# ypw0102/GDR

Hardware: AMD Instinct MI355X
Metric: queries/sec on NQ-320k (768-d) (higher is better)
Workload: dtype f32; 1 GPU; C2/ragged/prefilter: t5-base encoder 512 q/GPU + Q.D^T top-100, 320000x768 corpus; batch_per_gpu=512, global_batch=512, seq_len=40, corpus_rows=320000, dim=768, k=100, encoder_rows=ragged

## Files before the change

### gdr_amd/csrc/common.h

```cpp
#pragma once
#include <hip/hip_runtime.h>
#include <stdint.h>
#include <stdio.h>
#include <stdarg.h>
#include <stdlib.h>

#include "../../include/gdr_hip.h"

namespace gdr {

void set_error(const char* fmt, ...);

#define GDR_CHECK_ARG(cond, ...)                \
  do {                                          \
    if (!(cond)) {                              \
      gdr::set_error(__VA_ARGS__);              \
      return GDR_EINVAL;                        \
    }                                           \
  } while (0)

void count_launch();
#define GDR_CHECK_LAUNCH(what)                                                   \
  do {                                                                           \
    gdr::count_launch();                                                         \
// ... 29 lines not shown
  ~ProfScope();
};

constexpr int CNT_STRIDE = 32;
struct SimEpilogue {
  float* cand_val;
  int32_t* cand_idx;
  int32_t* cand_cnt;
  const float* thr;
  int32_t* status;
  int32_t cap;
  int32_t tile_stride;
  int32_t mode;
};

struct StreamK {
  float* part;
  int32_t* flag;
  int32_t epoch;
  const int32_t* live = nullptr;
};
constexpr size_t STREAMK_PART_BYTES = (size_t)512 * 128 * 128 * 4;
constexpr size_t STREAMK_BYTES = STREAMK_PART_BYTES + 4096;

enum { ACT_NONE = 0, ACT_RELU = 1, ACT_GELU = 2 };
struct LinearEpilogue {
  bool has_bias, has_residual;
  int act;
};
static inline bool decode_epilogue(int epilogue, LinearEpilogue* e) {
  if (epilogue < GDR_EPI_NONE || epilogue > GDR_EPI_BIAS_GELU) return false;
  e->has_bias = epilogue == GDR_EPI_BIAS || epilogue == GDR_EPI_BIAS_RELU || epilogue == GDR_EPI_BIAS_RESIDUAL ||
                epilogue == GDR_EPI_BIAS_GELU;
  e->has_residual = epilogue == GDR_EPI_RESIDUAL || epilogue == GDR_EPI_BIAS_RESIDUAL;
  e->act = (epilogue == GDR_EPI_RELU || epilogue == GDR_EPI_BIAS_RELU) ? ACT_RELU
           : epilogue == GDR_EPI_BIAS_GELU                             ? ACT_GELU
                                                                       : ACT_NONE;
  return true;
}

int launch_linear_f32(const float* A, int64_t lda, const float* W, int64_t ldw, float* C, int64_t ldc, int64_t M,
                      int N, int K, int epilogue, const float* bias, const float* residual, int64_t ldr,
                      hipStream_t stream);
int launch_linear_f32_ws(const float* A, int64_t lda, const float* W, int64_t ldw, float* C, int64_t ldc, int64_t M,
                         int N, int K, int epilogue, const float* bias, const float* residual, int64_t ldr,
                         float* splitk_ws, size_t splitk_ws_bytes, hipStream_t stream, StreamK* sk = nullptr,
                         const int64_t* m_dev = nullptr, int64_t prof_rows = -1);
int launch_linear_f32_ws_dev(const float* A, int64_t lda, const float* W, int64_t ldw, float* C, int64_t ldc, int64_t M_max,
                             const int64_t* m_dev, int N, int K, int epilogue, const float* bias, const float* residual,
                             int64_t ldr, float* splitk_ws, size_t splitk_ws_bytes, hipStream_t stream,
                             StreamK* sk = nullptr);
int launch_linear_f32_dev(const float* A, int64_t lda, const float* W, int64_t ldw, float* C, int64_t ldc, int64_t M_max,
                          const int64_t* m_dev, int N, int K, int epilogue, const float* bias, const float* residual,
                          int64_t ldr, int64_t prof_rows, hipStream_t stream, StreamK* sk = nullptr);
int launch_sim_gemm(const void* D, int64_t N, const void* Q, int B, int d, const SimEpilogue& ep, bool bf16,
                    hipStream_t stream);

int launch_linear_bf16(const void* A, int64_t lda, const void* W, int64_t ldw, float* C, int64_t ldc, int64_t M, int N,
                       int K, int epilogue, const float* bias, const float* residual, int64_t ldr, hipStream_t stream,
                       const int64_t* m_dev = nullptr);
struct NormEpilogue {
  int kind;
  const float *w1, *b1, *w2, *b2, *addv;
  float eps;
  float* Y;
  int64_t ldy;
  int y16_only = 0;
};
struct SlabRef {
  const float* part;
  int S, tiles_n;
};
int launch_linear_f32_small(const float* A, int64_t lda, const float* W, int64_t ldw, float* C, int64_t ldc, int64_t M, int N,
                            int K, int has_bias, int has_residual, int act, const float* bias, const float* residual,
                            int64_t ldr, float* ws, size_t ws_bytes, hipStream_t stream, const int64_t* m_dev = nullptr,
                            const NormEpilogue* ne = nullptr,
                            SlabRef* slabs = nullptr,
                            const int32_t* live = nullptr);
int linear_f32_small_splits(int64_t M, int N, int K, bool has_ws, size_t ws_bytes);
int launch_linear_bf16_headdot(const void* A, int64_t lda, const void* W, int64_t ldw, int64_t M, const int64_t* m_dev, int N, int K,
                               const float* h, int64_t ldh, const int32_t* rows_map, const float* E, int dot_d, float scale,
                               float* partial, hipStream_t stream);
int linear_bf16_tile_form(int64_t M, int N, int K, int has_residual, int out_bf16, int split = 0);
int launch_linear_bf16_glds(const void* A, int64_t lda, const void* W, int64_t ldw, float* C, int64_t ldc, int64_t M, int N,
                            int K, int has_bias, int has_residual, int act, const float* bias, const float* residual,
                            int64_t ldr, int out_bf16, hipStream_t stream, const int64_t* m_dev = nullptr,
                            int split = 0);
int split_row_elems(int K, int f16x2 = 0);
int launch_split_f32_bf16x3(const float* in, int64_t ld_in, void* out, int64_t ld_out, int64_t rows, int K, const int64_t* rows_dev,
                            hipStream_t stream, int f16x2 = 0);
int launch_sim_bf16_glds(const void* D, int64_t N, const void* Q, int B, int d, const SimEpilogue& ep, int64_t n_doc_tiles,
                         hipStream_t stream);
int launch_cast_f32_bf16(const float* in, void* out_bf16, int64_t n, hipStream_t stream);

bool sim_stream_supported(int B, int d, bool bf16);
int launch_sim_stream(const void* D, int64_t N, const void* Q, int B, int d, const SimEpilogue& ep, bool bf16, hipStream_t stream);

template <int CTRL>
__device__ __forceinline__ float dpp_row(float v) {
  return __builtin_bit_cast(float, __builtin_amdgcn_update_dpp(0, __builtin_bit_cast(int, v), CTRL, 0xF, 0xF, false));
}
__device__ __forceinline__ float row16_sum(float v) {
  v += dpp_row<0x128>(v);
  v += dpp_row<0x124>(v);
  v += dpp_row<0x122>(v);
  v += dpp_row<0x121>(v);
  return v;
// ... 32 lines not shown
```

### gdr_amd/csrc/common.hip

```cpp
#include <atomic>

#include "common.h"

#include <mutex>
#include <vector>

namespace gdr {
static thread_local char g_err[512] = "";

void set_error(const char* fmt, ...) {
  va_list ap;
  va_start(ap, fmt);
  vsnprintf(g_err, sizeof(g_err), fmt, ap);
  va_end(ap);
}

namespace {
struct AttrKey {
  const void* fn;
  int dev;
};
std::mutex g_attr_mu;
std::vector<AttrKey> g_attr_done;
}

int ensure_dyn_lds(const void* kernel, int bytes, const char* what) {
  int dev = 0;
  if (hipGetDevice(&dev) != hipSuccess) {
    set_error("%s: hipGetDevice failed", what);
    return GDR_EHIP;
  }
  std::lock_guard<std::mutex> lock(g_attr_mu);
  for (const AttrKey& k : g_attr_done)
    if (k.fn == kernel && k.dev == dev) return GDR_OK;
  hipError_t e = hipFuncSetAttribute(kernel, hipFuncAttributeMaxDynamicSharedMemorySize, bytes);
  if (e != hipSuccess) {
    set_error("%s: hipFuncSetAttribute: %s", what, hipGetErrorString(e));
    return GDR_EHIP;
  }
  g_attr_done.push_back(AttrKey{kernel, dev});
  return GDR_OK;
}

struct ProfState {
  bool on = false;
  bool gate = true;
  int cap = 0, used = 0;
  hipEvent_t* start = nullptr;
  hipEvent_t* stop = nullptr;
  int* cls = nullptr;
  double* work = nullptr;
};
static ProfState g_prof;

ProfScope::ProfScope(int c, double w, hipStream_t s) : slot(-1), stream(s) {
  if (!g_prof.on || !g_prof.gate || g_prof.used >= g_prof.cap) return;
  slot = g_prof.used++;
  g_prof.cls[slot] = c;
  g_prof.work[slot] = w;
  (void)hipEventRecord(g_prof.start[slot], stream);
}
ProfScope::~ProfScope() {
  if (slot >= 0) (void)hipEventRecord(g_prof.stop[slot], stream);
}
}

extern "C" void gdr_prof_gate(int on) { gdr::g_prof.gate = on != 0; }

extern "C" int gdr_prof_enable(int max_events) {
  using namespace gdr;
  if (g_prof.on || max_events <= 0) {
    set_error("prof_enable: already enabled or bad size");
    return GDR_EINVAL;
  }
  g_prof.start = new hipEvent_t[max_events];
  g_prof.stop = new hipEvent_t[max_events];
  g_prof.cls = new int[max_events];
  g_prof.work = new double[max_events];
  for (int i = 0; i < max_events; ++i) {
    if (hipEventCreate(&g_prof.start[i]) != hipSuccess || hipEventCreate(&g_prof.stop[i]) != hipSuccess) {
      set_error("prof_enable: hipEventCreate failed");
      return GDR_EHIP;
    }
  }
  g_prof.cap = max_events, g_prof.used = 0, g_prof.on = true;
  return GDR_OK;
}

extern "C" int gdr_prof_collect(int64_t* launches, double* total_ms, double* total_work) {
  using namespace gdr;
  if (!g_prof.on) {
    set_error("prof_collect: profiler not enabled");
    return GDR_EINVAL;
  }
  for (int c = 0; c < PROF_NCLASS; ++c) launches[c] = 0, total_ms[c] = 0.0, total_work[c] = 0.0;
  int rc = GDR_OK;
  for (int i = 0; i < g_prof.used; ++i) {
    float ms = 0.f;
    if (hipEventSynchronize(g_prof.stop[i]) != hipSuccess ||
        hipEventElapsedTime(&ms, g_prof.start[i], g_prof.stop[i]) != hipSuccess) {
      set_error("prof_collect: event query failed");
      rc = GDR_EHIP;
      break;
    }
    const int c = g_prof.cls[i];
    launches[c] += 1, total_ms[c] += ms, total_work[c] += g_prof.work[i];
  }
  for (int i = 0; i < g_prof.cap; ++i) {
    (void)hipEventDestroy(g_prof.start[i]);
    (void)hipEventDestroy(g_prof.stop[i]);
  }
  delete[] g_prof.start, delete[] g_prof.stop, delete[] g_prof.cls, delete[] g_prof.work;
  g_prof = ProfState();
  return rc;
}

namespace gdr {
static std::atomic<int64_t> g_launches{0};
void count_launch() { g_launches.fetch_add(1, std::memory_order_relaxed); }
}
extern "C" int64_t gdr_launch_count(void) { return gdr::g_launches.load(std::memory_order_relaxed); }
extern "C" const char* gdr_last_error(void) { return gdr::g_err; }
extern "C" int gdr_abi_version(void) { return 9; }
```

### gdr_amd/csrc/encoder.hip

```cpp
#include <stdlib.h>

#include "layers.h"

namespace gdr {

constexpr size_t ENC_SPLITK_BYTES = (size_t)112 << 20;
static_assert(STREAMK_BYTES <= ENC_SPLITK_BYTES, "stream-K scratch must fit the split-K region");
constexpr bool ENC_LAST_Q_CLS_DEFAULT = true;

static int enc_streamk(char* splitk_region, StreamK* sk, hipStream_t stream) {
  sk->part = reinterpret_cast<float*>(splitk_region);
  sk->flag = reinterpret_cast<int32_t*>(splitk_region + STREAMK_PART_BYTES);
  sk->epoch = 0;
  if (hipMemsetAsync(sk->flag, 0, 512 * sizeof(int32_t), stream) != hipSuccess) {
    set_error("t5_encoder: memset of the stream-K flags failed");
    return GDR_EHIP;
  }
  return GDR_OK;
}

struct EncWs {
  size_t off_h, off_nx, off_qkv, off_ctx, off_ff, off_splitk, off_bf, total;
};

static EncWs enc_ws(const GdrT5Dims& dm, int64_t M, bool bf16 = false) {
  EncWs w{};
  const size_t inner = (size_t)dm.num_heads * dm.d_kv;
  size_t o = 0;
  w.off_h = o, o += align_up((size_t)M * dm.d_model * 4, 256);
  w.off_nx = o, o += align_up((size_t)M * dm.d_model * 4, 256);
  w.off_qkv = o, o += align_up((size_t)M * 3 * inner * 4, 256);
  w.off_ctx = o, o += align_up((size_t)M * inner * 4, 256);
  w.off_ff = o, o += align_up((size_t)M * dm.d_ff * 4, 256);
  w.off_splitk = o, o += ENC_SPLITK_BYTES;
  w.off_bf = o;
  if (bf16) o += align_up((size_t)M * (dm.d_ff > dm.d_model ? dm.d_ff : dm.d_model) * 2, 256);
  w.total = o;
  return w;
}

}

extern "C" size_t gdr_t5_encoder_workspace_bytes(const GdrT5Dims* dims, int B, int L) {
  if (!dims || B <= 0 || L <= 0) return 0;
  return gdr::enc_ws(*dims, (int64_t)B * L).total;
}

namespace gdr {
static int t5_encoder_impl(const GdrT5EncoderWeights* w, const int64_t* ids, const int64_t* mask, int B, int L,
                           float* out_hidden, float* out_pooled, void* workspace, size_t workspace_bytes, bool bf16,
                           hipStream_t stream) {
  if (B == 0) return GDR_OK;
  GDR_CHECK_ARG(w && ids && out_hidden && workspace, "t5_encoder: null pointer");
// ... 73 lines not shown
      at.out_bf16 = abf;
      if ((rc = launch_attention(at, stream))) return rc;
      if ((rc = lin16(abf, ly.wo, h, d, d, inner, 0, h, 0))) return rc;
      if ((rc = launch_rmsnorm_bf16(h, ly.ln_ff, abf, M, d, dm.eps, stream))) return rc;
      if ((rc = lin16(abf, ly.wi, ff, dm.d_ff, dm.d_ff, d, 1, nullptr, 1))) return rc;
      if ((rc = lin16(ff, ly.wo_ff, h, d, d, dm.d_ff, 0, h, 0))) return rc;
      continue;
    }
    if ((rc = launch_rmsnorm(h, ly.ln_attn, nx, M, d, dm.eps, nullptr, 1, stream))) return rc;
    if ((rc = linear(nx, d, ly.wqkv, qkv, 3 * inner, 3 * inner, d, GDR_EPI_NONE, nullptr))) return rc;
    if ((rc = launch_attention(at, stream))) return rc;
    if ((rc = linear(ctx, inner, ly.wo, h, d, d, inner, GDR_EPI_RESIDUAL, h))) return rc;
    if ((rc = launch_rmsnorm(h, ly.ln_ff, nx, M, d, dm.eps, nullptr, 1, stream))) return rc;
    if ((rc = linear(nx, d, ly.wi, ff, dm.d_ff, dm.d_ff, d, GDR_EPI_RELU, nullptr))) return rc;
    if ((rc = linear(ff, dm.d_ff, ly.wo_ff, h, d, d, dm.d_ff, GDR_EPI_RESIDUAL, h))) return rc;
  }
  return launch_rmsnorm(h, w->final_ln, out_hidden, M, d, dm.eps, out_pooled, L, stream);
}
}

extern "C" int gdr_t5_encoder_forward(const GdrT5EncoderWeights* w, const int64_t* ids, const int64_t* mask, int B,
                                      int L, float* out_hidden, float* out_pooled, void* workspace,
                                      size_t workspace_bytes, void* stream_) {
  return gdr::t5_encoder_impl(w, ids, mask, B, L, out_hidden, out_pooled, workspace, workspace_bytes, false,
                              static_cast<hipStream_t>(stream_));
}

namespace gdr {
struct RagWs {
  size_t seq_len, seq_off, row_src, rows_total, ctx_cls, h_cls, nx_cls, ff_cls, total;
};
static RagWs rag_ws(const GdrT5Dims& dm, int B, int L, size_t base) {
  RagWs r{};
  const size_t inner = (size_t)dm.num_heads * dm.d_kv;
  size_t o = base;
  r.seq_len = o, o += align_up((size_t)B * 4, 256);
  r.seq_off = o, o += align_up((size_t)(B + 1) * 4, 256);
  r.row_src = o, o += align_up((size_t)B * L * 4, 256);
  r.rows_total = o, o += 256;
  r.ctx_cls = o, o += align_up((size_t)B * inner * 4, 256);
  r.h_cls = o, o += align_up((size_t)B * dm.d_model * 4, 256);
  r.nx_cls = o, o += align_up((size_t)B * dm.d_model * 4, 256);
  r.ff_cls = o, o += align_up((size_t)B * dm.d_ff * 4, 256);
  r.total = o;
  return r;
}
static bool ragged_packs(const GdrT5Dims& dm, int B, int L) {
  const int64_t tiles = (((int64_t)B * L + 127) / 128) * ((dm.d_model + 127) / 128);
  return dm.d_kv == 64 && tiles >= 192 && dm.d_model % 32 == 0 && dm.d_ff % 32 == 0 && (dm.num_heads * dm.d_kv) % 32 == 0;
}
static bool ragged_packs_small(const GdrT5Dims& dm, int B, int L) {
  return dm.d_kv == 64 && (int64_t)B * L >= 256 && dm.d_model % 32 == 0 && dm.d_ff % 32 == 0 && (dm.num_heads * dm.d_kv) % 32 == 0;
}
}

extern "C" size_t gdr_t5_encoder_ragged_workspace_bytes(const GdrT5Dims* dims, int B, int L) {
  if (!dims || B <= 0 || L <= 0) return 0;
  return gdr::rag_ws(*dims, B, L, gdr::enc_ws(*dims, (int64_t)B * L, true).total).total;
}

namespace gdr {
static int ragged_impl(const GdrT5EncoderWeights* w, const int64_t* ids, const int64_t* mask, int B, int L, float* out_hidden,
                       float* out_pooled, int64_t live_rows_hint, void* workspace, size_t workspace_bytes, bool bf16,
                       hipStream_t stream) {
  if (B == 0) return GDR_OK;
  GDR_CHECK_ARG(w && ids && mask && workspace && (out_hidden || out_pooled), "t5_encoder_ragged: null pointer");
  const GdrT5Dims& dm = w->dims;
  GDR_CHECK_ARG(B > 0 && L > 0 && L <= T5_MAX_LEN, "t5_encoder_ragged: B=%d L=%d (L must be in [1,%d])", B, L, T5_MAX_LEN);
  GDR_CHECK_ARG(dm.d_model % 4 == 0 && dm.d_kv % 4 == 0 && dm.d_ff % 4 == 0, "t5_encoder_ragged: dims must be multiples of 4");
  GDR_CHECK_ARG(w->embed && w->rel_bias && w->final_ln && w->layers, "t5_encoder_ragged: null weight pointer");
  const int64_t M = (int64_t)B * L;
  const EncWs ws = enc_ws(dm, M, true);
  const RagWs rw = rag_ws(dm, B, L, ws.total);
  if (workspace_bytes < rw.total) {
    set_error("t5_encoder_ragged: workspace %zu < required %zu", workspace_bytes, rw.total);
    return GDR_ENOSPC;
  }
  GDR_CHECK_ARG(((uintptr_t)workspace & 255) == 0, "t5_encoder_ragged: workspace must be 256-byte aligned");
  char* base = static_cast<char*>(workspace);
  const int d = dm.d_model, H = dm.num_heads, dk = dm.d_kv, inner = H * dk;
  int rc;
  int32_t* seq_len = reinterpret_cast<int32_t*>(base + rw.seq_len);
  int32_t* seq_off = reinterpret_cast<int32_t*>(base + rw.seq_off);
  int32_t* row_src = reinterpret_cast<int32_t*>(base + rw.row_src);
  int64_t* rows_dev = reinterpret_cast<int64_t*>(base + rw.rows_total);
  if ((rc = launch_pack_plan(mask, B, L, seq_len, seq_off, row_src, rows_dev, stream))) return rc;
  const bool fused16 = bf16 && d % 64 == 0 && inner % 64 == 0 && dm.d_ff % 64 == 0 && (((uintptr_t)w->layers[0].wqkv) & 15) == 0;
  const bool big = ragged_packs(dm, B, L);
  const bool small = !big && !bf16 && ragged_packs_small(dm, B, L);
  if ((!big && !small) || (bf16 && !fused16)) {
    float* full = out_hidden ? out_hidden : reinterpret_cast<float*>(base + ws.off_qkv);
    if ((rc = t5_encoder_impl(w, ids, mask, B, L, full, out_pooled, workspace, ws.total, bf16, stream))) return rc;
    return out_hidden ? launch_zero_dead_rows(out_hidden, seq_len, B, L, d, stream) : GDR_OK;
  }
  if (bf16) {
    float* h = reinterpret_cast<float*>(base + ws.off_h);
    float* nx = reinterpret_cast<float*>(base + ws.off_nx);
    float* qkv = reinterpret_cast<float*>(base + ws.off_qkv);
    float* ff = reinterpret_cast<float*>(base + ws.off_ff);
    void* abf = base + ws.off_bf;
    float* h_cls = reinterpret_cast<float*>(base + rw.h_cls);
    void* ctx_cls16 = base + rw.ctx_cls;
    void* nx_cls16 = base + rw.nx_cls;
    void* ff_cls16 = base + rw.ff_cls;
    auto lin16 = [&](const void* A, const float* W, float* C, int64_t ldc, int64_t rows, const int64_t* md, int N, int K, int act,
                     const float* residual, int out_bf16) -> int {
      ProfScope prof(PROF_LINEAR, 2.0 * (double)(md && live_rows_hint >= 0 ? live_rows_hint : rows) * (double)N * (double)K, stream);
      const int rc_ = launch_linear_bf16_glds(A, K, W, K, C, ldc, rows, N, K, 0, residual != nullptr, act, nullptr, residual, ldc,
                                              out_bf16, stream, md);
      if (rc_ > 0) {
        set_error("t5_encoder_ragged_bf16: shape not served by the LDS-DMA linear");
        return GDR_EINVAL;
      }
      return rc_;
    };
    if ((rc = launch_embed_packed(w->embed, ids, row_src, rows_dev, M, d, dm.vocab_size, h, stream))) return rc;
    AttnArgs at{};
    const bool qkv16 = L <= 128;
    if (qkv16) {
      const __bf16* q16 = reinterpret_cast<const __bf16*>(qkv);
      at.q = reinterpret_cast<const float*>(q16), at.k = reinterpret_cast<const float*>(q16 + inner);
      at.v = reinterpret_cast<const float*>(q16 + 2 * inner), at.qkv_bf16 = 1;
    } else {
      at.q = qkv, at.k = qkv + inner, at.v = qkv + 2 * inner;
    }
    at.out = nullptr, at.out_bf16 = abf;
    at.ldq = at.ldk = at.ldv = 3 * inner, at.ldo = inner;
    at.q_bstride = at.k_bstride = at.o_bstride = L;
    at.B = B, at.H = H, at.dk = dk, at.Lq = L, at.Lk = L;
    at.q_pos0 = 0, at.scale = 1.0f;
    at.rel_bias = w->rel_bias, at.bidirectional = 1, at.num_buckets = dm.rel_buckets;
    at.lut = make_bucket_lut(dm.rel_buckets / 2, dm.rel_max_distance);
    at.key_mask = mask, at.mask_bstride = L, at.causal = 0, at.causal_neg_inf = 0;
    at.kv_rows = nullptr, at.kv_group = 1;
    at.seq_off = seq_off, at.seq_len = seq_len;
    const bool pooled_only = out_hidden == nullptr;
    for (int i = 0; i < dm.num_layers; ++i) {
      const GdrT5EncLayer& ly = w->layers[i];
      GDR_CHECK_ARG(ly.ln_attn && ly.wqkv && ly.wo && ly.ln_ff && ly.wi && ly.wo_ff, "t5_encoder_ragged: layer %d null weight", i);
      if ((rc = launch_rmsnorm_bf16_dev(h, ly.ln_attn, abf, rows_dev, M, d, dm.eps, stream))) return rc;
      if ((rc = lin16(abf, ly.wqkv, qkv, 3 * inner, M, rows_dev, 3 * inner, d, 0, nullptr, qkv16 ? 1 : 0))) return rc;
      if ((rc = launch_attention(at, stream))) return rc;
      if (pooled_only && i == dm.num_layers - 1) {
        if ((rc = launch_gather_rows(static_cast<const float*>(abf), seq_off, B, inner / 2, static_cast<float*>(ctx_cls16), stream)))
          return rc;
        if ((rc = launch_gather_rows(h, seq_off, B, d, h_cls, stream))) return rc;
        if ((rc = lin16(ctx_cls16, ly.wo, h_cls, d, B, nullptr, d, inner, 0, h_cls, 0))) return rc;
        if ((rc = launch_rmsnorm_bf16(h_cls, ly.ln_ff, nx_cls16, B, d, dm.eps, stream))) return rc;
        if ((rc = lin16(nx_cls16, ly.wi, static_cast<float*>(ff_cls16), dm.d_ff, B, nullptr, dm.d_ff, d, 1, nullptr, 1))) return rc;
        if ((rc = lin16(ff_cls16, ly.wo_ff, h_cls, d, B, nullptr, d, dm.d_ff, 0, h_cls, 0))) return rc;
        return launch_rmsnorm(h_cls, w->final_ln, out_pooled, B, d, dm.eps, nullptr, 1, stream);
      }
      if ((rc = lin16(abf, ly.wo, h, d, M, rows_dev, d, inner, 0, h, 0))) return rc;
      if ((rc = launch_rmsnorm_bf16_dev(h, ly.ln_ff, abf, rows_dev, M, d, dm.eps, stream))) return rc;
      if ((rc = lin16(abf, ly.wi, ff, dm.d_ff, M, rows_dev, dm.d_ff, d, 1, nullptr, 1))) return rc;
      if ((rc = lin16(ff, ly.wo_ff, h, d, M, rows_dev, d, dm.d_ff, 0, h, 0))) return rc;
    }
    if ((rc = launch_rmsnorm_dev(h, w->final_ln, nx, rows_dev, M, d, dm.eps, stream))) return rc;
    if (out_pooled && (rc = launch_gather_rows(nx, seq_off, B, d, out_pooled, stream))) return rc;
    if (out_hidden) {
      if (hipMemsetAsync(out_hidden, 0, (size_t)M * d * sizeof(float), stream) != hipSuccess) {
        set_error("t5_encoder_ragged: memset failed");
        return GDR_EHIP;
      }
      if ((rc = launch_scatter_rows(nx, row_src, rows_dev, M, d, out_hidden, stream))) return rc;
    }
    return GDR_OK;
  }
  float* h = reinterpret_cast<float*>(base + ws.off_h);
  float* nx = reinterpret_cast<float*>(base + ws.off_nx);
  float* qkv = reinterpret_cast<float*>(base + ws.off_qkv);
  float* ctx = reinterpret_cast<float*>(base + ws.off_ctx);
  float* ff = reinterpret_cast<float*>(base + ws.off_ff);
  float* ctx_cls = reinterpret_cast<float*>(base + rw.ctx_cls);
  float* h_cls = reinterpret_cast<float*>(base + rw.h_cls);
  float* nx_cls = reinterpret_cast<float*>(base + rw.nx_cls);
  float* ff_cls = reinterpret_cast<float*>(base + rw.ff_cls);
  StreamK sk{};
  if ((rc = enc_streamk(base + ws.off_splitk, &sk, stream))) return rc;
  float* skw = reinterpret_cast<float*>(base + ws.off_splitk);
  auto linear = [&](const float* A, int64_t lda, const float* W, float* C, int64_t ldc, int N, int K, int epi,
                    const float* residual) -> int {
    if (small)
      return launch_linear_f32_ws(A, lda, W, K, C, ldc, M, N, K, epi, nullptr, residual, ldc, skw, ENC_SPLITK_BYTES, stream, &sk,
                                  rows_dev, live_rows_hint);
    return launch_linear_f32_dev(A, lda, W, K, C, ldc, M, rows_dev, N, K, epi, nullptr, residual, ldc, live_rows_hint, stream,
                                 &sk);
  };
  const float* qkv0 = big ? w->qkv0_table : nullptr;
  GDR_CHECK_ARG(!qkv0 || (((uintptr_t)qkv0) & 15) == 0, "t5_encoder_ragged: qkv0_table must be 16-byte aligned");
  if (qkv0)
    rc = launch_embed_packed2(w->embed, qkv0, ids, row_src, rows_dev, M, d, 3 * inner, dm.vocab_size, h, qkv, stream);
  else
    rc = launch_embed_packed(w->embed, ids, row_src, rows_dev, M, d, dm.vocab_size, h, stream);
  if (rc) return rc;

  AttnArgs at{};
  at.q = qkv, at.k = qkv + inner, at.v = qkv + 2 * inner, at.out = ctx;
  at.ldq = at.ldk = at.ldv = 3 * inner, at.ldo = inner;
  at.q_bstride = at.k_bstride = at.o_bstride = L;
  at.B = B, at.H = H, at.dk = dk, at.Lq = L, at.Lk = L;
  at.q_pos0 = 0, at.scale = 1.0f;
  at.rel_bias = w->rel_bias, at.bidirectional = 1, at.num_buckets = dm.rel_buckets;
  at.lut = make_bucket_lut(dm.rel_buckets / 2, dm.rel_max_distance);
  at.key_mask = mask, at.mask_bstride = L, at.causal = 0, at.causal_neg_inf = 0;
  at.kv_rows = nullptr, at.kv_group = 1;
  at.seq_off = seq_off, at.seq_len = seq_len;

  const bool pooled_only = out_hidden == nullptr && big;
  static const bool last_q_cls_on = [] {
    const char* e = getenv("GDR_ENC_LAST_Q_CLS");
    return e ? atoi(e) != 0 : ENC_LAST_Q_CLS_DEFAULT;
  }();
  for (int i = 0; i < dm.num_layers; ++i) {
    const GdrT5EncLayer& ly = w->layers[i];
    GDR_CHECK_ARG(ly.ln_attn && ly.wqkv && ly.wo && ly.ln_ff && ly.wi && ly.wo_ff, "t5_encoder_ragged: layer %d null weight", i);
    if (i == 0 && qkv0) {
    } else if (pooled_only && i == dm.num_layers - 1 && last_q_cls_on) {
      if ((rc = launch_rmsnorm_dev(h, ly.ln_attn, nx, rows_dev, M, d, dm.eps, stream))) return rc;
      if ((rc = linear(nx, d, ly.wqkv + (size_t)inner * d, qkv + inner, 3 * inner, 2 * inner, d, GDR_EPI_NONE, nullptr))) return rc;
      if ((rc = launch_gather_rows(nx, seq_off, B, d, nx_cls, stream))) return rc;
      if ((rc = launch_linear_f32(nx_cls, d, ly.wqkv, d, ctx_cls, inner, B, inner, d, GDR_EPI_NONE, nullptr, nullptr, 0, stream)))
        return rc;
      if ((rc = launch_scatter_rows_strided(ctx_cls, seq_off, B, inner, qkv, 3 * inner, stream))) return rc;
    } else {
      if ((rc = launch_rmsnorm_dev(h, ly.ln_attn, nx, rows_dev, M, d, dm.eps, stream))) return rc;
      if ((rc = linear(nx, d, ly.wqkv, qkv, 3 * inner, 3 * inner, d, GDR_EPI_NONE, nullptr))) return rc;
    }
    if ((rc = launch_attention(at, stream))) return rc;
    if (pooled_only && i == dm.num_layers - 1) {
      if ((rc = launch_gather_rows(ctx, seq_off, B, inner, ctx_cls, stream))) return rc;
      if ((rc = launch_gather_rows(h, seq_off, B, d, h_cls, stream))) return rc;
      if ((rc = launch_linear_f32(ctx_cls, inner, ly.wo, inner, h_cls, d, B, d, inner, GDR_EPI_RESIDUAL, nullptr, h_cls, d, stream)))
        return rc;
      if ((rc = launch_rmsnorm(h_cls, ly.ln_ff, nx_cls, B, d, dm.eps, nullptr, 1, stream))) return rc;
      if ((rc = launch_linear_f32(nx_cls, d, ly.wi, d, ff_cls, dm.d_ff, B, dm.d_ff, d, GDR_EPI_RELU, nullptr, nullptr, 0, stream)))
        return rc;
      if ((rc = launch_linear_f32(ff_cls, dm.d_ff, ly.wo_ff, dm.d_ff, h_cls, d, B, d, dm.d_ff, GDR_EPI_RESIDUAL, nullptr, h_cls, d,
                                  stream)))
        return rc;
// ... 196 lines not shown
```

### gdr_amd/csrc/gemm_f32.hip

```cpp
#include <stdlib.h>

#include "common.h"

namespace gdr {

typedef float f32x16 __attribute__((ext_vector_type(16)));
typedef float f32x4 __attribute__((ext_vector_type(4)));
typedef __bf16 bf16x8_t __attribute__((ext_vector_type(8)));

constexpr int BM = 128, BN = 128, BK = 32;
constexpr int LDS_STRIDE = BK + 4;
constexpr int GEMM_THREADS = 256;

struct GemmArgs {
  const float* A;
  const float* W;
  float* C;
  const float* bias;
  const float* residual;
  int64_t lda, ldw, ldc, ldr;
  int64_t M;
  int N, K;
  int tiles_n;
  int has_bias, has_residual, act;
// ... 819 lines not shown
  float4 v = *reinterpret_cast<const float4*>(p);
  int s = 1;
  for (; s + 4 <= S; s += 4) {
    const float4 t0 = *reinterpret_cast<const float4*>(p + (int64_t)(s + 0) * (BM * BN));
    const float4 t1 = *reinterpret_cast<const float4*>(p + (int64_t)(s + 1) * (BM * BN));
    const float4 t2 = *reinterpret_cast<const float4*>(p + (int64_t)(s + 2) * (BM * BN));
    const float4 t3 = *reinterpret_cast<const float4*>(p + (int64_t)(s + 3) * (BM * BN));
    v.x += t0.x, v.y += t0.y, v.z += t0.z, v.w += t0.w;
    v.x += t1.x, v.y += t1.y, v.z += t1.z, v.w += t1.w;
    v.x += t2.x, v.y += t2.y, v.z += t2.z, v.w += t2.w;
    v.x += t3.x, v.y += t3.y, v.z += t3.z, v.w += t3.w;
  }
  for (; s < S; ++s) {
    const float4 t = *reinterpret_cast<const float4*>(p + (int64_t)s * (BM * BN));
    v.x += t.x, v.y += t.y, v.z += t.z, v.w += t.w;
  }
  float o[4] = {v.x, v.y, v.z, v.w};
#pragma unroll
  for (int q = 0; q < 4; ++q) {
    if (n + q >= N) break;
    float x = o[q];
    if (bias) x += bias[n + q];
    if (residual) x += residual[m * ldr + n + q];
    if (act == ACT_RELU) x = fmaxf(x, 0.f);
    if (act == ACT_GELU) x = gelu_erf(x);
    C[m * ldc + n + q] = x;
  }
}

enum LinearForm {
  FORM_NONE = 0,
  FORM_TILES,
  FORM_PERSISTENT,
  FORM_SMALL,
  FORM_SPLITK,
  FORM_STREAMK_UNITS,
  FORM_STREAMK_256,
  FORM_STREAMK_TAIL
};
struct LinearRoute {
  LinearForm form;
  int slabs, chunk_steps;
  int grid;
};
struct LinearCall {
  int64_t M;
  int N, K;
  int64_t lda, ldw;
  size_t ws_bytes;
  bool has_sk;
  bool dev_rows;
  int64_t row_hint;
  bool whole_k;
};
static LinearRoute linear_f32_route(const LinearCall& c) {
  if (c.M <= 0 || c.N <= 0 || c.K <= 0 || c.K % 4 != 0) return {FORM_NONE, 0, 0, 0};
  const int tiles_n = (c.N + BN - 1) / BN;
  const int64_t tiles = ((c.M + BM - 1) / BM) * tiles_n;
  const int nk = c.K / BK;
  const bool kfull = c.K % BK == 0;
  if (!c.whole_k && tiles < 192 && nk >= 4 && kfull) {
    if (c.M <= 1536) {
      const int S = linear_f32_small_splits(c.M, c.N, c.K, c.ws_bytes > 0, c.ws_bytes);
      if (S) return {FORM_SMALL, S, 0, 0};
    }
    const int S = linear_f32_splitk_slabs(tiles, nk, c.ws_bytes);
    if (S >= 2) {
      const int chunk_steps = (nk + S - 1) / S, S2 = (nk + chunk_steps - 1) / chunk_steps;
      const int64_t units_hint = c.dev_rows && c.row_hint >= 0 ? ((c.row_hint + BM - 1) / BM) * tiles_n * S2 : -1;
      const size_t need = STREAMK_BYTES + (size_t)tiles * S2 * BM * BN * sizeof(float);
      const bool units = c.has_sk && c.dev_rows && nk % chunk_steps == 0 && tiles * S2 > 256 && (units_hint < 0 || units_hint > 256) &&
                         need <= c.ws_bytes && streamk_fits(c.M, c.lda, c.N, c.ldw);
      return {units ? FORM_STREAMK_UNITS : FORM_SPLITK, S2, chunk_steps, units ? 256 : 0};
    }
  }
  const int64_t tiles_adm = c.whole_k && c.row_hint >= 0 ? ((c.row_hint + BM - 1) / BM) * tiles_n : tiles;
  const bool sk_ok = c.has_sk && kfull && streamk_fits(c.M, c.lda, c.N, c.ldw);
  if (sk_ok && tiles > 256 && streamk_mid_wanted(tiles_adm)) return {FORM_STREAMK_256, 0, 0, 256};
  if (tiles > 512 && tiles < 0x7fffffff && kfull)
    return {sk_ok && streamk_wanted(tiles_adm, nk) ? FORM_STREAMK_TAIL : FORM_PERSISTENT, 0, 0, 512};
  return {FORM_TILES, 0, 0, 0};
}

static int supertile_height(int tiles_n) { return tiles_n >= 12 ? 8 : 1; }

static int build_linear_args(const char* what, int mult, const void* A, int64_t lda, const void* W, int64_t ldw, float* C,
                             int64_t ldc, int64_t M, int N, int K, int epilogue, const float* bias, const float* residual,
                             int64_t ldr, const int64_t* m_dev, GemmArgs* g) {
  GDR_CHECK_ARG(A && W && C, "%s: null pointer", what);
  GDR_CHECK_ARG(M >= 0 && N > 0 && K > 0, "%s: bad shape M=%lld N=%d K=%d", what, (long long)M, N, K);
  GDR_CHECK_ARG(K % mult == 0 && lda % mult == 0 && ldw % mult == 0, "%s: K, lda, ldw must be multiples of %d", what, mult);
  GDR_CHECK_ARG(lda >= K && ldw >= K && ldc >= N, "%s: leading dimension smaller than the row", what);
  GDR_CHECK_ARG(aligned16(A) && aligned16(W), "%s: A and W must be 16-byte aligned", what);
  LinearEpilogue e;
  GDR_CHECK_ARG(decode_epilogue(epilogue, &e), "%s: unknown epilogue %d", what, epilogue);
  GDR_CHECK_ARG(!e.has_bias || bias, "%s: epilogue %d needs bias", what, epilogue);
  GDR_CHECK_ARG(!e.has_residual || (residual && ldr >= N), "%s: epilogue %d needs residual", what, epilogue);
  *g = GemmArgs{};
  g->A = static_cast<const float*>(A), g->W = static_cast<const float*>(W);
  g->C = C, g->bias = bias, g->residual = residual;
  g->lda = lda, g->ldw = ldw, g->ldc = ldc, g->ldr = ldr;
  g->M = M, g->N = N, g->K = K, g->m_dev = m_dev;
  g->tiles_n = (N + BN - 1) / BN;
  g->has_bias = e.has_bias, g->has_residual = e.has_residual, g->act = e.act;
  return GDR_OK;
}

template <bool UNITS>
static int launch_streamk(const GemmArgs& g, int64_t items, int grid, StreamK* sk, int S, float* slabs, const char* what,
                          hipStream_t stream) {
  GDR_TRY(streamk_poll_error());
  const StreamKArgs ska{sk->part, sk->flag, ++sk->epoch, streamk_err_word(), S, slabs};
  hipLaunchKernelGGL(gemm_nt_f32_streamk_kernel<UNITS>, dim3((unsigned)grid), dim3(GEMM_THREADS), 0, stream, g, (int)items, ska);
  GDR_CHECK_LAUNCH(what);
  return GDR_OK;
}

static int launch_whole_k(GemmArgs& g, const LinearRoute& r, StreamK* sk, hipStream_t stream) {
  const int64_t tiles_m = (g.M + BM - 1) / BM, tiles = tiles_m * g.tiles_n;
  switch (r.form) {
    case FORM_STREAMK_256:
    case FORM_STREAMK_TAIL:
      g.ksplit = supertile_height(g.tiles_n);
      return launch_streamk<false>(g, tiles, r.grid, sk, 0, nullptr,
                                   r.grid == 256 ? "gemm_nt_f32_streamk_kernel(256)" : "gemm_nt_f32_streamk_kernel", stream);
    case FORM_PERSISTENT:
      g.ksplit = supertile_height(g.tiles_n);
      hipLaunchKernelGGL(gemm_nt_f32_persistent_kernel, dim3((unsigned)r.grid), dim3(GEMM_THREADS), 0, stream, g, (int)tiles);
      GDR_CHECK_LAUNCH("gemm_nt_f32_persistent_kernel");
      return GDR_OK;
// ... 15 lines not shown
  if (M == 0) return GDR_OK;
  GemmArgs g;
  GDR_TRY(build_linear_args("linear", 4, A, lda, W, ldw, C, ldc, M, N, K, epilogue, bias, residual, ldr, m_dev, &g));
  LinearRoute r = linear_f32_route({M, N, K, lda, ldw, splitk_ws ? splitk_ws_bytes : 0, sk != nullptr, m_dev != nullptr, prof_rows, false});
  if (r.form == FORM_STREAMK_UNITS && sk->part != splitk_ws) r.form = FORM_SPLITK;
  const double flops = 2.0 * (double)(m_dev && prof_rows >= 0 ? prof_rows : M) * (double)N * (double)K;
  if (r.form == FORM_SMALL)
    return launch_linear_f32_small(A, lda, W, ldw, C, ldc, M, N, K, g.has_bias, g.has_residual, g.act, bias, residual, ldr, splitk_ws,
                                   splitk_ws_bytes, stream, m_dev, nullptr, nullptr, sk ? sk->live : nullptr);
  if (r.form == FORM_SPLITK || r.form == FORM_STREAMK_UNITS) {
    const int64_t tiles = ((M + BM - 1) / BM) * g.tiles_n;
    float* slabs = r.form == FORM_SPLITK ? splitk_ws : reinterpret_cast<float*>(reinterpret_cast<char*>(splitk_ws) + STREAMK_BYTES);
    GemmArgs p = g;
    p.C = slabs, p.has_bias = 0, p.has_residual = 0, p.act = ACT_NONE;
    p.kchunk = r.chunk_steps * BK, p.tile_base = 0;
    if (r.form == FORM_SPLITK) {
      p.ksplit = r.slabs;
      {
        ProfScope prof(PROF_LINEAR, flops, stream);
        hipLaunchKernelGGL(gemm_nt_f32_kernel<EPI_LINEAR>, dim3((unsigned)(tiles * r.slabs)), dim3(GEMM_THREADS), 0, stream, p);
      }
      GDR_CHECK_LAUNCH("gemm_nt_f32_kernel(split)");
    } else {
      p.ksplit = 1;
      ProfScope prof(PROF_LINEAR, flops, stream);
      GDR_TRY(launch_streamk<true>(p, tiles * r.slabs, r.grid, sk, r.slabs, slabs, "gemm_nt_f32_streamk_kernel(units)", stream));
    }
    ProfScope prof_r(PROF_REDUCE, 0.0, stream);
    hipLaunchKernelGGL(splitk_reduce_kernel, dim3((unsigned)(tiles * 16)), dim3(256), 0, stream, slabs, r.slabs, 0, g.tiles_n, M, N,
                       C, ldc, g.has_bias ? bias : nullptr, g.has_residual ? residual : nullptr, ldr, g.act, m_dev);
    GDR_CHECK_LAUNCH("splitk_reduce_kernel");
    return GDR_OK;
  }
  ProfScope prof(PROF_LINEAR, flops, stream);
  return launch_whole_k(g, r, sk, stream);
}

int launch_linear_f32_ws_dev(const float* A, int64_t lda, const float* W, int64_t ldw, float* C, int64_t ldc, int64_t M_max,
                             const int64_t* m_dev, int N, int K, int epilogue, const float* bias, const float* residual,
                             int64_t ldr, float* splitk_ws, size_t splitk_ws_bytes, hipStream_t stream, StreamK* sk) {
  if (M_max == 0) return GDR_OK;
  GDR_CHECK_ARG(m_dev, "linear(dev rows): null row count");
  const LinearRoute r = linear_f32_route({M_max, N, K, lda, ldw, splitk_ws ? splitk_ws_bytes : 0, sk != nullptr, true, -1, false});
  if (r.form != FORM_SMALL)
    return launch_linear_f32_dev(A, lda, W, ldw, C, ldc, M_max, m_dev, N, K, epilogue, bias, residual, ldr, -1, stream, sk);
  GemmArgs g;
  GDR_TRY(build_linear_args("linear(dev rows)", 4, A, lda, W, ldw, C, ldc, M_max, N, K, epilogue, bias, residual, ldr, m_dev, &g));
  return launch_linear_f32_small(A, lda, W, ldw, C, ldc, M_max, N, K, g.has_bias, g.has_residual, g.act, bias, residual, ldr, splitk_ws,
                                 splitk_ws_bytes, stream, m_dev, nullptr, nullptr, sk ? sk->live : nullptr);
}

int launch_linear_f32_dev(const float* A, int64_t lda, const float* W, int64_t ldw, float* C, int64_t ldc, int64_t M_max,
                          const int64_t* m_dev, int N, int K, int epilogue, const float* bias, const float* residual,
                          int64_t ldr, int64_t prof_rows, hipStream_t stream, StreamK* sk) {
  if (M_max == 0) return GDR_OK;
  GDR_CHECK_ARG(m_dev, "linear(dev rows): null row count");
  GemmArgs g;
  GDR_TRY(build_linear_args("linear(dev rows)", 4, A, lda, W, ldw, C, ldc, M_max, N, K, epilogue, bias, residual, ldr, m_dev, &g));
  GDR_CHECK_ARG(M_max > 0 && K % BK == 0, "linear(dev rows): bad shape M<=%lld N=%d K=%d (K %% 32 == 0)", (long long)M_max, N, K);
  GDR_CHECK_ARG(((M_max + BM - 1) / BM) * g.tiles_n < 0x7fffffff, "linear(dev rows): grid too large");
  ProfScope prof(PROF_LINEAR, 2.0 * (double)(prof_rows >= 0 ? prof_rows : M_max) * (double)N * (double)K, stream);
  return launch_whole_k(g, linear_f32_route({M_max, N, K, lda, ldw, 0, sk != nullptr, true, prof_rows, true}), sk, stream);
}

int launch_linear_bf16(const void* A, int64_t lda, const void* W, int64_t ldw, float* C, int64_t ldc, int64_t M, int N,
                       int K, int epilogue, const float* bias, const float* residual, int64_t ldr, hipStream_t stream,
                       const int64_t* m_dev) {
  if (M == 0) return GDR_OK;
  GemmArgs g;
  GDR_TRY(build_linear_args("linear_bf16", 8, A, lda, W, ldw, C, ldc, M, N, K, epilogue, bias, residual, ldr, m_dev, &g));
  ProfScope prof(PROF_LINEAR, 2.0 * (double)M * (double)N * (double)K, stream);
  {
    const int rc = launch_linear_bf16_glds(A, lda, W, ldw, C, ldc, M, N, K, g.has_bias, g.has_residual, g.act, bias, residual, ldr, 0,
                                           stream, m_dev);
    if (rc <= 0) return rc;
  }
  return launch<EPI_LINEAR, true>(g, (M + BM - 1) / BM, stream);
}

int launch_sim_gemm(const void* D_, int64_t N, const void* Q_, int B, int d, const SimEpilogue& ep, bool bf16,
                    hipStream_t stream) {
  const float* D = static_cast<const float*>(D_);
  const float* Q = static_cast<const float*>(Q_);
  GemmArgs g{};
  g.A = D, g.W = Q, g.lda = d, g.ldw = d;
  g.M = N, g.N = B, g.K = d;
  g.tiles_n = (B + BN - 1) / BN;
  g.sim = ep;
  const int64_t tiles_m = (N + BM - 1) / BM;
  const int64_t n_sample_tiles = (tiles_m + ep.tile_stride - 1) / ep.tile_stride;
  if (ep.mode == 1) {
    int64_t rows = n_sample_tiles * BM;
    if (rows > N) rows = N;
    ProfScope prof(PROF_SIM_SAMPLE, 2.0 * (double)rows * (double)B * (double)d, stream);
    if (bf16) {
      const int rc = launch_sim_bf16_glds(D_, N, Q_, B, d, ep, n_sample_tiles, stream);
      if (rc <= 0) return rc;
    }
    return bf16 ? launch<EPI_SIM_SAMPLE, true>(g, n_sample_tiles, stream) : launch<EPI_SIM_SAMPLE>(g, n_sample_tiles, stream);
  }
  int64_t rows = (tiles_m - n_sample_tiles) * BM;
  if (rows > N) rows = N;
  ProfScope prof(PROF_SIM_FILTER, 2.0 * (double)rows * (double)B * (double)d, stream);
  if (bf16) {
    const int rc = launch_sim_bf16_glds(D_, N, Q_, B, d, ep, tiles_m - n_sample_tiles, stream);
    if (rc <= 0) return rc;
  }
  return bf16 ? launch<EPI_SIM_FILTER, true>(g, tiles_m - n_sample_tiles, stream)
              : launch<EPI_SIM_FILTER>(g, tiles_m - n_sample_tiles, stream);
}

}

extern "C" int gdr_linear_f32(const float* A, int64_t lda, const float* W, int64_t ldw, float* C, int64_t ldc,
                              int64_t M, int N, int K, int epilogue, const float* bias, const float* residual,
// ... 51 lines not shown
```

Baseline: 31200 queries/s.

## Split ragged encoder batch into two concurrent stream chains with capped GEMM grids

The ragged T5 encoder now splits the batch in half and runs each half on its own stream (main plus a pooled side stream). An optional stagger event delays the second chain by a few linears. Each chain's linears use a persistent or stream-K grid capped at 256 so the two chains can share the GPU, which targets idle compute during small or serial kernels like attention and norms. The workspace grows to hold two chains, and the profiler now merges overlapping spans per class so it does not double-count concurrent time.

```diff
diff --git a/gdr_amd/csrc/common.h b/gdr_amd/csrc/common.h
--- a/gdr_amd/csrc/common.h
+++ b/gdr_amd/csrc/common.h
@@ -105,7 +105,7 @@
                              StreamK* sk = nullptr);
 int launch_linear_f32_dev(const float* A, int64_t lda, const float* W, int64_t ldw, float* C, int64_t ldc, int64_t M_max,
                           const int64_t* m_dev, int N, int K, int epilogue, const float* bias, const float* residual,
-                          int64_t ldr, int64_t prof_rows, hipStream_t stream, StreamK* sk = nullptr);
+                          int64_t ldr, int64_t prof_rows, hipStream_t stream, StreamK* sk = nullptr, int grid_cap = 0);
 int launch_sim_gemm(const void* D, int64_t N, const void* Q, int B, int d, const SimEpilogue& ep, bool bf16,
                     hipStream_t stream);
 
diff --git a/gdr_amd/csrc/common.hip b/gdr_amd/csrc/common.hip
--- a/gdr_amd/csrc/common.hip
+++ b/gdr_amd/csrc/common.hip
@@ -1,3 +1,4 @@
+#include <algorithm>
 #include <atomic>
 
 #include "common.h"
@@ -95,16 +96,37 @@
   }
   for (int c = 0; c < PROF_NCLASS; ++c) launches[c] = 0, total_ms[c] = 0.0, total_work[c] = 0.0;
   int rc = GDR_OK;
+  struct Span {
+    double t0, t1;
+  };
+  std::vector<Span> spans[PROF_NCLASS];
+  double anchor_t = 0.0;
+  int anchor = 0;
   for (int i = 0; i < g_prof.used; ++i) {
-    float ms = 0.f;
+    float ms = 0.f, rel = 0.f;
     if (hipEventSynchronize(g_prof.stop[i]) != hipSuccess ||
-        hipEventElapsedTime(&ms, g_prof.start[i], g_prof.stop[i]) != hipSuccess) {
+        hipEventElapsedTime(&ms, g_prof.start[i], g_prof.stop[i]) != hipSuccess ||
+        (i != anchor && hipEventElapsedTime(&rel, g_prof.start[anchor], g_prof.start[i]) != hipSuccess)) {
       set_error("prof_collect: event query failed");
       rc = GDR_EHIP;
       break;
     }
+    const double t0 = anchor_t + (double)rel;
+    if (i - anchor >= 64) anchor = i, anchor_t = t0;
     const int c = g_prof.cls[i];
-    launches[c] += 1, total_ms[c] += ms, total_work[c] += g_prof.work[i];
+    launches[c] += 1, total_work[c] += g_prof.work[i];
+    spans[c].push_back(Span{t0, t0 + (double)ms});
+  }
+  for (int c = 0; c < PROF_NCLASS && rc == GDR_OK; ++c) {
+    std::sort(spans[c].begin(), spans[c].end(), [](const Span& a, const Span& b) { return a.t0 < b.t0; });
+    double end = 0.0;
+    for (size_t i = 0; i < spans[c].size(); ++i) {
+      const Span& s = spans[c][i];
+      if (i == 0 || s.t0 >= end)
+        total_ms[c] += s.t1 - s.t0, end = s.t1;
+      else if (s.t1 > end)
+        total_ms[c] += s.t1 - end, end = s.t1;
+    }
   }
   for (int i = 0; i < g_prof.cap; ++i) {
     (void)hipEventDestroy(g_prof.start[i]);
diff --git a/gdr_amd/csrc/encoder.hip b/gdr_amd/csrc/encoder.hip
--- a/gdr_amd/csrc/encoder.hip
+++ b/gdr_amd/csrc/encoder.hip
@@ -1,4 +1,7 @@
 #include <stdlib.h>
+
+#include <mutex>
+#include <vector>
 
 #include "layers.h"
 
@@ -178,17 +181,106 @@
 static bool ragged_packs_small(const GdrT5Dims& dm, int B, int L) {
   return dm.d_kv == 64 && (int64_t)B * L >= 256 && dm.d_model % 32 == 0 && dm.d_ff % 32 == 0 && (dm.num_heads * dm.d_kv) % 32 == 0;
 }
+
+constexpr int ENC_CHAIN_GRID = 256;
+constexpr int ENC_CHAINS_DEFAULT = 2;
+constexpr int ENC_CHAIN_STAGGER_DEFAULT = 1;
+struct EncChain {
+  int grid_cap;
+  hipEvent_t after;
+  int after_linears;
+};
+static bool enc_chains_eligible(const GdrT5Dims& dm, int B, int L) {
+  return B >= 2 && dm.num_layers >= 2 && ragged_packs(dm, B / 2, L);
+}
+static size_t ragged_one_chain_bytes(const GdrT5Dims& dm, int B, int L) {
+  return rag_ws(dm, B, L, enc_ws(dm, (int64_t)B * L, true).total).total;
+}
+static size_t ragged_bytes(const GdrT5Dims& dm, int B, int L) {
+  const size_t one = ragged_one_chain_bytes(dm, B, L);
+  if (!enc_chains_eligible(dm, B, L)) return one;
+  const size_t two = ragged_one_chain_bytes(dm, B / 2, L) + ragged_one_chain_bytes(dm, B - B / 2, L);
+  return two > one ? two : one;
+}
+
+struct EncSide {
+  hipStream_t s = nullptr;
+  hipEvent_t fork = nullptr, stagger = nullptr, join = nullptr;
+  int dev = -1;
+};
+static std::mutex g_enc_side_mu;
+static std::vector<EncSide*> g_enc_side_free;
+static EncSide* enc_side_acquire() {
+  int dev = 0;
+  if (hipGetDevice(&dev) != hipSuccess) return nullptr;
+  {
+    std::lock_guard<std::mutex> lock(g_enc_side_mu);
+    for (size_t i = 0; i < g_enc_side_free.size(); ++i)
+      if (g_enc_side_free[i]->dev == dev) {
+        EncSide* x = g_enc_side_free[i];
+        g_enc_side_free.erase(g_enc_side_free.begin() + i);
+        return x;
+      }
+  }
+  EncSide* x = new EncSide();
+  x->dev = dev;
+  if (hipStreamCreateWithFlags(&x->s, hipStreamNonBlocking) != hipSuccess ||
+      hipEventCreateWithFlags(&x->fork, hipEventDisableTiming) != hipSuccess ||
+      hipEventCreateWithFlags(&x->stagger, hipEventDisableTiming) != hipSuccess ||
+      hipEventCreateWithFlags(&x->join, hipEventDisableTiming) != hipSuccess) {
+    (void)hipGetLastError();
+    delete x;
+    return nullptr;
+  }
+  return x;
+}
+static void enc_side_release(EncSide* x) {
+  std::lock_guard<std::mutex> lock(g_enc_side_mu);
+  g_enc_side_free.push_back(x);
+}
+
+static int ragged_impl(const GdrT5EncoderWeights* w, const int64_t* ids, const int64_t* mask, int B, int L, float* out_hidden,
+                       float* out_pooled, int64_t live_rows_hint, void* workspace, size_t workspace_bytes, bool bf16,
+                       hipStream_t stream, const EncChain* chain = nullptr);
+
+static int ragged_two_chains(const GdrT5EncoderWeights* w, const int64_t* ids, const int64_t* mask, int B, int L, float* out_pooled,
+                             int64_t live_rows_hint, char* base, int stagger, EncSide* side, hipStream_t stream) {
+  const GdrT5Dims& dm = w->dims;
+  const int BA = B / 2, BB = B - BA;
+  const size_t bytes_a = ragged_one_chain_bytes(dm, BA, L), bytes_b = ragged_one_chain_bytes(dm, BB, L);
+  const int64_t hint_a = live_rows_hint >= 0 ? live_rows_hint / 2 : -1;
+  const int64_t hint_b = live_rows_hint >= 0 ? live_rows_hint - hint_a : -1;
+  if (hipEventRecord(side->fork, stream) != hipSuccess || hipStreamWaitEvent(side->s, side->fork, 0) != hipSuccess) {
+    set_error("t5_encoder_ragged: fork to the side stream failed");
+    return GDR_EHIP;
+  }
+  const EncChain ca{ENC_CHAIN_GRID, stagger > 0 ? side->stagger : nullptr, stagger};
+  const EncChain cb{ENC_CHAIN_GRID, nullptr, 0};
+  int rc = ragged_impl(w, ids, mask, BA, L, nullptr, out_pooled, hint_a, base, bytes_a, false, stream, &ca);
+  if (rc == GDR_OK && stagger > 0 && hipStreamWaitEvent(side->s, side->stagger, 0) != hipSuccess) {
+    set_error("t5_encoder_ragged: wait on the stagger event failed");
+    rc = GDR_EHIP;
+  }
+  if (rc == GDR_OK)
+    rc = ragged_impl(w, ids + (size_t)BA * L, mask + (size_t)BA * L, BB, L, nullptr, out_pooled + (size_t)BA * dm.d_model, hint_b,
+                     base + bytes_a, bytes_b, false, side->s, &cb);
+  if (hipEventRecord(side->join, side->s) != hipSuccess || hipStreamWaitEvent(stream, side->join, 0) != hipSuccess) {
+    if (rc == GDR_OK) set_error("t5_encoder_ragged: join of the side stream failed");
+    return rc ? rc : GDR_EHIP;
+  }
+  return rc;
+}
 }
 
 extern "C" size_t gdr_t5_encoder_ragged_workspace_bytes(const GdrT5Dims* dims, int B, int L) {
   if (!dims || B <= 0 || L <= 0) return 0;
-  return gdr::rag_ws(*dims, B, L, gdr::enc_ws(*dims, (int64_t)B * L, true).total).total;
+  return gdr::ragged_bytes(*dims, B, L);
 }
 
 namespace gdr {
 static int ragged_impl(const GdrT5EncoderWeights* w, const int64_t* ids, const int64_t* mask, int B, int L, float* out_hidden,
                        float* out_pooled, int64_t live_rows_hint, void* workspace, size_t workspace_bytes, bool bf16,
-                       hipStream_t stream) {
+                       hipStream_t stream, const EncChain* chain) {
   if (B == 0) return GDR_OK;
   GDR_CHECK_ARG(w && ids && mask && workspace && (out_hidden || out_pooled), "t5_encoder_ragged: null pointer");
   const GdrT5Dims& dm = w->dims;
@@ -198,12 +290,31 @@
   const int64_t M = (int64_t)B * L;
   const EncWs ws = enc_ws(dm, M, true);
   const RagWs rw = rag_ws(dm, B, L, ws.total);
-  if (workspace_bytes < rw.total) {
-    set_error("t5_encoder_ragged: workspace %zu < required %zu", workspace_bytes, rw.total);
+  const size_t required = chain ? rw.total : ragged_bytes(dm, B, L);
+  if (workspace_bytes < required) {
+    set_error("t5_encoder_ragged: workspace %zu < required %zu", workspace_bytes, required);
     return GDR_ENOSPC;
   }
   GDR_CHECK_ARG(((uintptr_t)workspace & 255) == 0, "t5_encoder_ragged: workspace must be 256-byte aligned");
   char* base = static_cast<char*>(workspace);
+  if (!chain && !bf16 && !out_hidden && enc_chains_eligible(dm, B, L)) {
+    static const int chains = [] {
+      const char* e = getenv("GDR_ENC_CHAINS");
+      return e ? atoi(e) : ENC_CHAINS_DEFAULT;
+    }();
+    static const int stagger = [] {
+      const char* e = getenv("GDR_ENC_CHAIN_STAGGER");
+      const int v = e ? atoi(e) : ENC_CHAIN_STAGGER_DEFAULT;
+      return v < 0 ? 0 : v > 3 ? 3 : v;
+    }();
+    if (chains == 2) {
+      if (EncSide* side = enc_side_acquire()) {
+        const int rc2 = ragged_two_chains(w, ids, mask, B, L, out_pooled, live_rows_hint, base, stagger, side, stream);
+        enc_side_release(side);
+        return rc2;
+      }
+    }
+  }
   const int d = dm.d_model, H = dm.num_heads, dk = dm.d_kv, inner = H * dk;
   int rc;
   int32_t* seq_len = reinterpret_cast<int32_t*>(base + rw.seq_len);
@@ -305,13 +416,19 @@
   StreamK sk{};
   if ((rc = enc_streamk(base + ws.off_splitk, &sk, stream))) return rc;
   float* skw = reinterpret_cast<float*>(base + ws.off_splitk);
+  int batch_linears = 0;
   auto linear = [&](const float* A, int64_t lda, const float* W, float* C, int64_t ldc, int N, int K, int epi,
                     const float* residual) -> int {
     if (small)
       return launch_linear_f32_ws(A, lda, W, K, C, ldc, M, N, K, epi, nullptr, residual, ldc, skw, ENC_SPLITK_BYTES, stream, &sk,
                                   rows_dev, live_rows_hint);
-    return launch_linear_f32_dev(A, lda, W, K, C, ldc, M, rows_dev, N, K, epi, nullptr, residual, ldc, live_rows_hint, stream,
-                                 &sk);
+    GDR_TRY(launch_linear_f32_dev(A, lda, W, K, C, ldc, M, rows_dev, N, K, epi, nullptr, residual, ldc, live_rows_hint, stream, &sk,
+                                  chain ? chain->grid_cap : 0));
+    if (chain && chain->after && ++batch_linears == chain->after_linears && hipEventRecord(chain->after, stream) != hipSuccess) {
+      set_error("t5_encoder_ragged: event record behind a linear failed");
+      return GDR_EHIP;
+    }
+    return GDR_OK;
   };
   const float* qkv0 = big ? w->qkv0_table : nullptr;
   GDR_CHECK_ARG(!qkv0 || (((uintptr_t)qkv0) & 15) == 0, "t5_encoder_ragged: qkv0_table must be 16-byte aligned");
diff --git a/gdr_amd/csrc/gemm_f32.hip b/gdr_amd/csrc/gemm_f32.hip
--- a/gdr_amd/csrc/gemm_f32.hip
+++ b/gdr_amd/csrc/gemm_f32.hip
@@ -895,6 +895,7 @@
   bool dev_rows;
   int64_t row_hint;
   bool whole_k;
+  int grid_cap = 0;
 };
 static LinearRoute linear_f32_route(const LinearCall& c) {
   if (c.M <= 0 || c.N <= 0 || c.K <= 0 || c.K % 4 != 0) return {FORM_NONE, 0, 0, 0};
@@ -919,6 +920,8 @@
   }
   const int64_t tiles_adm = c.whole_k && c.row_hint >= 0 ? ((c.row_hint + BM - 1) / BM) * tiles_n : tiles;
   const bool sk_ok = c.has_sk && kfull && streamk_fits(c.M, c.lda, c.N, c.ldw);
+  if (c.whole_k && c.grid_cap > 0 && tiles > c.grid_cap && tiles < 0x7fffffff && kfull)
+    return {sk_ok ? FORM_STREAMK_TAIL : FORM_PERSISTENT, 0, 0, c.grid_cap};
   if (sk_ok && tiles > 256 && streamk_mid_wanted(tiles_adm)) return {FORM_STREAMK_256, 0, 0, 256};
   if (tiles > 512 && tiles < 0x7fffffff && kfull)
     return {sk_ok && streamk_wanted(tiles_adm, nk) ? FORM_STREAMK_TAIL : FORM_PERSISTENT, 0, 0, 512};
@@ -1040,7 +1043,7 @@
 
 int launch_linear_f32_dev(const float* A, int64_t lda, const float* W, int64_t ldw, float* C, int64_t ldc, int64_t M_max,
                           const int64_t* m_dev, int N, int K, int epilogue, const float* bias, const float* residual,
-                          int64_t ldr, int64_t prof_rows, hipStream_t stream, StreamK* sk) {
+                          int64_t ldr, int64_t prof_rows, hipStream_t stream, StreamK* sk, int grid_cap) {
   if (M_max == 0) return GDR_OK;
   GDR_CHECK_ARG(m_dev, "linear(dev rows): null row count");
   GemmArgs g;
@@ -1048,7 +1051,7 @@
   GDR_CHECK_ARG(M_max > 0 && K % BK == 0, "linear(dev rows): bad shape M<=%lld N=%d K=%d (K %% 32 == 0)", (long long)M_max, N, K);
   GDR_CHECK_ARG(((M_max + BM - 1) / BM) * g.tiles_n < 0x7fffffff, "linear(dev rows): grid too large");
   ProfScope prof(PROF_LINEAR, 2.0 * (double)(prof_rows >= 0 ? prof_rows : M_max) * (double)N * (double)K, stream);
-  return launch_whole_k(g, linear_f32_route({M_max, N, K, lda, ldw, 0, sk != nullptr, true, prof_rows, true}), sk, stream);
+  return launch_whole_k(g, linear_f32_route({M_max, N, K, lda, ldw, 0, sk != nullptr, true, prof_rows, true, grid_cap}), sk, stream);
 }
 
 int launch_linear_bf16(const void* A, int64_t lda, const void* W, int64_t ldw, float* C, int64_t ldc, int64_t M, int N,
```

Result: faster. 32060 queries/s, median of 6 (+2.8%).
